# Qiyuan-Ge/PaintMind

Measured on AMD Instinct MI355X. Metric: 256x256 images/sec, 8-step MaskGIT decode (vit-s-vqgan), whole job, higher is better.
Workload: dtype bf16; 1 GPU; maskgit-uncond-12L-d512-T8; batch_per_gpu=64, topk=5, decode=every step (reference-equivalent work), parallelism=dp1 (independent images, no data-path collective), hip_graph=True, concurrent_micro_batches=2, dispatch_mode=AMD_DIRECT_DISPATCH=1 (default), rank_mode=False

## Files before the change

include/pmhip.h:

```cpp
#ifndef PMHIP_H
#define PMHIP_H

#include <stdint.h>

#ifdef __cplusplus
extern "C" {
#endif

#define PMHIP_ABI_VERSION 11

enum { PMHIP_OK = 0, PMHIP_EINVAL = 1, PMHIP_EHIP = 2, PMHIP_ENOMEM = 3, PMHIP_ESTATE = 4 };
enum { PMHIP_F32 = 0, PMHIP_BF16 = 1 };
enum { PMHIP_PART_Q = 0, PMHIP_PART_K = 1, PMHIP_PART_V = 2 };

typedef void* pmhip_stream;

int pmhip_abi_version(void);
const char* pmhip_last_error(void);
int pmhip_device_info(int device, int* cu_count, int* lds_bytes, char* arch, int arch_len);


int pmhip_gemm(int dtype, const void* A, int lda, const void* W, int ldw, const float* bias,
               const float* residual, int ldr, int res_rows, void* out, int ldo, int out_dtype,
               int M, int N, int K, pmhip_stream stream);
// ... 34 lines not shown
    const float* parts; int nparts; float eps;
} pmhip_lnfold;

int pmhip_gemm_ln(int dtype, const void* A, int lda, const void* W, int ldw, const float* bias, void* out,
                  int ldo, int out_dtype, int M, int N, int K, const pmhip_lnfold* ln, pmhip_stream stream);
int pmhip_gemm_swiglu_ln(int dtype, const void* A, int lda, const void* W12p, const float* b12p, void* out,
                         int ldo, int M, int Hp, int K, const pmhip_lnfold* ln, pmhip_stream stream);
int pmhip_gemm_heads_ln(int dtype, const void* A, int lda, const void* W, int ldw, int M, int K, int heads,
                        int tokens, int tokens_pad, int nparts, const int* part_kinds_host,
                        void* const* part_outs_host, float q_scale, const pmhip_lnfold* ln,
                        pmhip_stream stream);
int pmhip_lnfold_supported(int dtype, int epi_kind, int M, int N, int K);

int pmhip_gemm_softmax_stats(int dtype, const void* A, int lda, const void* W, int ldw, const float* bias, float* out, int ldo,
                             int M, int N, int K, const pmhip_lnfold* ln, float* block_stats, pmhip_stream stream);

int pmhip_attention(int dtype, const void* Q, const void* K, const void* Vt, void* out, int ldo,
                    int B, int heads, int Nq, int Nkv, int Nkv_pad, int use_exp2,
                    pmhip_stream stream);

int pmhip_attention_fallbacks(unsigned long long* count, int reset);

int pmhip_gemm_heads_dh(int dtype, const void* A, int lda, const void* W, int ldw, int M, int K, int heads, int dim_head,
                        int tokens, int tokens_pad, int nparts, const int* part_kinds_host,
                        void* const* part_outs_host, float q_scale, float* scratch, pmhip_stream stream);
int pmhip_attention_dh(int dtype, const void* Q, const void* K, const void* Vt, void* out, int ldo, int B, int heads,
                       int dim_head, int Nq, int Nkv, int Nkv_pad, int use_exp2, pmhip_stream stream);

int pmhip_layernorm(const float* x, const float* gamma, const float* beta, float eps, void* out,
                    int out_dtype, int M, int D, pmhip_stream stream);
// ... 175 lines not shown
                                   uint64_t image_base, float* imgs_out, int use_graph,
                                   pmhip_stream stream, float* imgs_host, size_t host_stride,
                                   pmhip_stream copy_stream, float guidance_scale);

#define PMHIP_SLOTS_GRAPH        1
#define PMHIP_SLOTS_KEEP_CONTEXT 2
int pmhip_pipeline_step_slots(pmhip_s2* s2, int64_t* ids, const float* context, int L, int B,
                              const pmhip_slot* slots_host, int flags,
                              int64_t* pred_out, float* score_out, pmhip_stream stream);

int pmhip_pipeline_step_slots_guided(pmhip_s2* s2, int64_t* ids, const float* context, int L, int B,
                                     const pmhip_slot* slots_host, const pmhip_slot_guide* guides_host, int flags,
                                     int64_t* pred_out, float* score_out, pmhip_stream stream);

int pmhip_s2_switches(const pmhip_s2* h);
int pmhip_vqgan_switches(const pmhip_vqgan* h);
int pmhip_s2_step0_shared(const pmhip_s2* h, int* fills, int* hits);
int pmhip_s2_slots_steps(const pmhip_s2* h, int* one_pass, int* two_pass);

int pmhip_timing_enable(int on);
int pmhip_timing_reset(void);
int pmhip_timing_get(const char* family, int* launches, double* total_ms);

#ifdef __cplusplus
}
#endif
#endif
```

paintmind_amd/_lib.py:

```python
import ctypes as C
import os

_HERE = os.path.dirname(os.path.abspath(__file__))
LIB_PATH = os.path.join(_HERE, "libpaintmind_hip.so")

PMHIP_OK = 0
PMHIP_EINVAL, PMHIP_EHIP, PMHIP_ENOMEM, PMHIP_ESTATE = 1, 2, 3, 4
F32, BF16 = 0, 1
PART_Q, PART_K, PART_V = 0, 1, 2
ABI_VERSION = 11
GENERATE_GRAPH, GENERATE_CONCURRENT_LANES, GENERATE_FROM_MASK = 1, 2, 4
SLOTS_GRAPH, SLOTS_KEEP_CONTEXT = 1, 2
SLOT_IDLE = 0x80000000

vp = C.c_void_p
i32 = C.c_int
f32 = C.c_float
u64 = C.c_uint64
u32 = C.c_uint32
i64 = C.c_int64


class LayerWeights(C.Structure):
    _fields_ = [(n, vp) for n in (
# ... 51 lines not shown
    "pmhip_gemm_swiglu": (i32, [i32, vp, i32, vp, vp, vp, i32, i32, i32, i32, vp]),
    "pmhip_gemm_heads": (i32, [i32, vp, i32, vp, i32, i32, i32, i32, i32, i32, i32, C.POINTER(i32),
                               C.POINTER(vp), f32, vp]),
    "pmhip_gemm_hilo": (i32, [vp, i32, vp, i32, vp, vp, vp, i32, i32, vp, vp, i32, i32, i32, i32, vp]),
    "pmhip_gemm_hilo_stats": (i32, [vp, i32, vp, i32, vp, vp, vp, i32, i32, vp, vp, i32, i32, i32, i32, vp, vp]),
    "pmhip_gemm_hilo_center": (i32, [vp, i32, vp, i32, vp, vp, vp, i32, i32, vp, vp, i32, i32, i32, i32, vp, vp, C.c_float, vp, i32, vp]),
    "pmhip_unshift_hilo": (i32, [vp, vp, vp, i32, i32, vp]),
    "pmhip_ln_coef_parts": (i32, [vp, i32, f32, vp, i32, vp]),
    "pmhip_layernorm_hilo": (i32, [vp, vp, vp, vp, f32, vp, i32, i32, i32, vp]),
    "pmhip_layernorm_to_hilo": (i32, [vp, vp, vp, f32, vp, vp, i32, i32, vp]),
    "pmhip_split_hilo": (i32, [vp, vp, vp, i32, i32, vp]),
    "pmhip_join_hilo": (i32, [vp, vp, vp, i32, i32, vp]),
    "pmhip_ln_coef": (i32, [vp, f32, vp, i32, i32, vp]),
    "pmhip_gemm_ln": (i32, [i32, vp, i32, vp, i32, vp, vp, i32, i32, i32, i32, i32, C.POINTER(LnFold), vp]),
    "pmhip_gemm_softmax_stats": (i32, [i32, vp, i32, vp, i32, vp, vp, i32, i32, i32, i32, C.POINTER(LnFold), vp, vp]),
    "pmhip_gemm_swiglu_ln": (i32, [i32, vp, i32, vp, vp, vp, i32, i32, i32, i32, C.POINTER(LnFold), vp]),
    "pmhip_gemm_heads_ln": (i32, [i32, vp, i32, vp, i32, i32, i32, i32, i32, i32, i32, C.POINTER(i32),
                                  C.POINTER(vp), f32, C.POINTER(LnFold), vp]),
    "pmhip_lnfold_supported": (i32, [i32, i32, i32, i32, i32]),
    "pmhip_attention": (i32, [i32, vp, vp, vp, vp, i32, i32, i32, i32, i32, i32, i32, vp]),
    "pmhip_attention_fallbacks": (i32, [C.POINTER(C.c_ulonglong), i32]),
    "pmhip_gemm_heads_dh": (i32, [i32, vp, i32, vp, i32, i32, i32, i32, i32, i32, i32, i32, C.POINTER(i32),
                                  C.POINTER(vp), f32, vp, vp]),
    "pmhip_attention_dh": (i32, [i32, vp, vp, vp, vp, i32, i32, i32, i32, i32, i32, i32, i32, vp]),
    "pmhip_layernorm": (i32, [vp, vp, vp, f32, vp, i32, i32, i32, vp]),
    "pmhip_patchify": (i32, [vp, vp, i32, i32, i32, i32, i32, i32, vp]),
    "pmhip_unpatchify_clamp": (i32, [vp, vp, i32, i32, i32, i32, i32, f32, f32, vp]),
    "pmhip_convert_pad": (i32, [vp, i32, vp, i32, i32, i32, vp]),
    "pmhip_add_rows": (i32, [vp, vp, i32, vp, i32, i32, vp]),
    "pmhip_guidance_combine": (i32, [vp, vp, C.c_float, vp, C.c_size_t, vp]),
# ... 74 lines not shown
```

paintmind_amd/csrc/engine.hip:

```cpp
#include <stdarg.h>
#include <string.h>

#include <algorithm>
#include <cmath>
#include <atomic>
#include <map>
#include <memory>
#include <mutex>

#include "common.h"

static thread_local std::string g_err;

void pm_set_error(const char* fmt, ...) {
    char buf[1024];
    va_list ap;
    va_start(ap, fmt);
    vsnprintf(buf, sizeof buf, fmt, ap);
    va_end(ap);
    g_err = buf;
}

extern "C" const char* pmhip_last_error(void) { return g_err.c_str(); }
extern "C" int pmhip_abi_version(void) { return PMHIP_ABI_VERSION; }
// ... 145 lines not shown
constexpr float kLog2e = 1.4426950408889634f;

struct CrossKV {
    const void* k = nullptr;
    const void* vt = nullptr;
    int L = 0, Lp = 0;
};

struct Switches {
    int overlap_rows = 65536;
    bool hilo = true;
    bool fold = true;
    int fold_rows_cap = 0;
    bool center = true;
    bool logits_stats = true;
    bool blocking_wait = false;
    static Switches from_env() {
        Switches w;
        const char* e = getenv("PMHIP_HILO");
        w.hilo = !(e && atoi(e) == 0);
        e = getenv("PMHIP_LN_UNFOLD");
        w.fold = !(e && atoi(e) != 0);
        e = getenv("PMHIP_FOLD_MAX_ROWS");
        w.fold_rows_cap = e ? atoi(e) : 0;
        e = getenv("PMHIP_HILO_CENTER");
        w.center = !(e && atoi(e) == 0);
        e = getenv("PMHIP_BLOCKING_WAIT");
        w.blocking_wait = e && atoi(e) != 0;
        e = getenv("PMHIP_DECODE_OVERLAP_MAX_ROWS");
        if (e) w.overlap_rows = atoi(e);
        w.logits_stats = pm_dev_knob("PMHIP_LOGITS_STATS", 1) != 0;
        return w;
    }
    int key() const { return (hilo ? 2 : 0) + (fold ? 1 : 0) + 4 + (center ? 8 : 0); }
};

struct FoldState {
    enum { kStale, kDeferred, kWritten } coef = kStale;
    bool parts = false;
    void produced(bool with_parts) { coef = kStale; parts = with_parts; }
    bool requested() { coef = parts ? kDeferred : kWritten; return !parts; }
    void consumed() { coef = kWritten; }
};

struct TowerBufs {
    float* x = nullptr;
// ... 506 lines not shown
    const size_t per = (size_t)B * heads * Lp * dh * es;
    unsigned char* kv;
    WS(h->ws, "ctx.kv", per * 2 * c.tower.depth, kv);
    float* split = nullptr;
    if (dh != 64) WS(h->ws, "ctx.split", (size_t)Mc * 2 * inner * 4, split);
    const int kinds[2] = {PMHIP_PART_K, PMHIP_PART_V};
    for (int l = 0; l < c.tower.depth; ++l) {
        void* outs[2] = {kv + per * (2 * l), kv + per * (2 * l + 1)};
        const unsigned char* wkv = reinterpret_cast<const unsigned char*>(h->layers[l].wqkv2) + (size_t)inner * dim * es;
        PM_TRY(pmhip_gemm_heads_dh(h->dtype, cp, dim, wkv, dim, Mc, dim, heads, dh, L, Lp, 2, kinds, outs, 1.0f, split, s));
        h->cross[l].k = outs[0]; h->cross[l].vt = outs[1]; h->cross[l].L = L; h->cross[l].Lp = Lp;
    }
    return PMHIP_OK;
}

int s2_tower(pmhip_s2* h, const void* tp, int B, float* logits, hipStream_t s, bool use_cross = true, float* block_stats = nullptr) {
    const auto& c = h->cfg;
    const int M = B * c.tokens, dim = c.tower.dim;
    TowerBufs tb;
    PM_TRY(alloc_tower(h->ws, h->sw, "s2", h->dtype, c.tower, B, c.tokens, tb, s));
    ResSrc pos;
    PM_TRY(pos_source(h->ws, "pos", tb.hilo, h->w.pos, c.tokens, dim, h->pos_split, pos, s));
    PM_TRY(residual_gemm(h->dtype, tb, tp, 64, h->w.tokproj_w, 64, h->w.tokproj_b, pos, M, dim, 64, s));
    for (int l = 0; l < c.tower.depth; ++l)
        PM_TRY(layer_forward(h->dtype, h->layers[l], c.tower, tb, B, c.tokens, true, use_cross ? &h->cross[l] : nullptr, s));
    if (tb.fold && h->w.logits_wf && fold_shape_ok(c.tokens, c.n_embed, dim))
        return folded_consumer(tb, M, c.tokens, dim, h->w.logits_c, h->w.logits_d, s, [&](int m0, int rows, const void* a, const pmhip_lnfold* ln) {
            float* out = logits + (size_t)m0 * c.n_embed;
            if (block_stats)
                return pmhip_gemm_softmax_stats(h->dtype, a, dim, h->w.logits_wf, dim, h->w.logits_b, out, c.n_embed, rows, c.n_embed, dim, ln,
                                                block_stats + (size_t)m0 * (c.n_embed / 64) * 2, s);
            return pmhip_gemm_ln(h->dtype, a, dim, h->w.logits_wf, dim, h->w.logits_b, out, c.n_embed, PMHIP_F32, rows, c.n_embed, dim, ln, s);
        });
    PM_TRY(tower_layernorm(h->dtype, tb, h->w.norm_g, h->w.norm_b, M, dim, s));
    if (block_stats)
        return pmhip_gemm_softmax_stats(h->dtype, tb.y, dim, h->w.logits_w, dim, h->w.logits_b, logits, c.n_embed, M, c.n_embed, dim, nullptr,
                                        block_stats, s);
    return pmhip_gemm(h->dtype, tb.y, dim, h->w.logits_w, dim, h->w.logits_b, nullptr, 0, 0, logits, c.n_embed, PMHIP_F32, M,
                      c.n_embed, dim, s);
}

struct StepBufs {
    float* logits = nullptr; float* lstats = nullptr;
    int64_t* pred = nullptr; float* score = nullptr;
};

int pred_bufs(pmhip_s2* s2, size_t M, StepBufs& b, hipStream_t s) {
    WS(s2->ws, "s2.pred", M * 8, b.pred);
    WS(s2->ws, "s2.score", M * 4, b.score);
    return PMHIP_OK;
}

int step_bufs(pmhip_s2* s2, int M, bool shared0, StepBufs& b, hipStream_t s) {
    const auto& c = s2->cfg;
    const size_t rows = shared0 ? c.tokens : M;
    WS(s2->ws, shared0 ? "s0.logits" : "s2.logits", rows * c.n_embed * 4, b.logits);
    b.lstats = nullptr;
    if (c.n_embed % 64 == 0 && s2->sw.logits_stats) WS(s2->ws, shared0 ? "s0.lstats" : "s2.lstats", rows * (c.n_embed / 64) * 8, b.lstats);
    return pred_bufs(s2, (size_t)M, b, s);
}

int tok_buf(pmhip_s2* s2, int M, void*& tp, hipStream_t s) {
    WS(s2->ws, "s2.tok", (size_t)M * 64 * dtype_size(s2->dtype), tp);
    return PMHIP_OK;
}

int step_tokens(pmhip_s2* s2, const int64_t* ids, int M, void*& tp, hipStream_t s) {
    PM_TRY(tok_buf(s2, M, tp, s));
    return pmhip_embed_rows(s2->w.tok_table, ids, tp, s2->dtype, 64, M, s2->cfg.n_embed + 1, s2->cfg.embed_dim, s);
}

int copy_aux(const StepBufs& b, size_t M, int64_t* pred_out, float* score_out, hipStream_t s) {
    if (pred_out) PM_HIP(hipMemcpyAsync(pred_out, b.pred, M * 8, hipMemcpyDeviceToDevice, s));
    if (score_out) PM_HIP(hipMemcpyAsync(score_out, b.score, M * 4, hipMemcpyDeviceToDevice, s));
    return PMHIP_OK;
}

int step_tower(pmhip_s2* s2, const int64_t* ids, int B, hipStream_t s, const float* guidance, const pmhip_slot* slots = nullptr,
               const pmhip_slot_guide* guides = nullptr) {
    const auto& c = s2->cfg;
    const int M = B * c.tokens;
    void* tp; StepBufs b;
    PM_TRY(step_tokens(s2, ids, M, tp, s));
    PM_TRY(step_bufs(s2, M, false, b, s));
    PM_TRY(s2_tower(s2, tp, B, b.logits, s, true, guidance ? nullptr : b.lstats));
    if (!guidance && !guides) return PMHIP_OK;
    float* uncond;
    WS(s2->ws, "s2.logits_u", (size_t)M * c.n_embed * 4, uncond);
    PM_TRY(s2_tower(s2, tp, B, uncond, s, false));
    if (guides) return pmhip_guidance_combine_slots(b.logits, uncond, guides, slots, c.tokens, b.logits, b.lstats, M, c.n_embed, s);
    if (b.lstats) return pmhip_guidance_combine_stats(b.logits, uncond, *guidance, b.logits, (size_t)M * c.n_embed, b.lstats, s);
    return pmhip_guidance_combine(b.logits, uncond, *guidance, b.logits, (size_t)M * c.n_embed, s);
}

int decode_pred(pmhip_s2* s2, pmhip_vqgan* vq, int B, float* img_out, hipStream_t s) {
    PM_REQUIRE(vq, "pipeline_sample: img_out requested without a vqgan handle");
    StepBufs b;
    PM_TRY(pred_bufs(s2, (size_t)B * s2->cfg.tokens, b, s));
    return vq_decode_indices(vq, b.pred, B, img_out, s);
}
// ... 218 lines not shown
    if (vq) img_elems = (size_t)B * vq->cfg.channels * vq->cfg.image_size * vq->cfg.image_size;
    int n_dec = 0;
    for (int t = 0; t < T; ++t) n_dec += c.decodes(t) ? 1 : 0;
    PM_REQUIRE(n_dec == 0 || (vq && (c.imgs_out || c.imgs_host)), "pipeline_generate: decode requested without vqgan / an image destination");
    PM_REQUIRE(!c.imgs_host || c.host_stride >= img_elems, "pipeline_generate: host_stride smaller than one image batch");
    const bool graph = (c.use_graph & PMHIP_GENERATE_GRAPH) && !g_pm_timing_on.load() && T <= PM_MAX_STEPS && !direct_dispatch_off();
    const bool from_mask = (c.use_graph & PMHIP_GENERATE_FROM_MASK) != 0;
    const bool share0 = from_mask && !c.context && !c.guidance && !g_pm_timing_on.load();
    const size_t n_ids = (size_t)B * s2->cfg.tokens;
    if (share0 && s2->s0_valid) {
        ++s2->s0_hits;
        if (s != s2->s0_stream) PM_HIP(hipStreamWaitEvent(s, s2->s0_ready.h, 0));
    }
    auto tower = [&](const int64_t* from, int t, hipStream_t on) -> int {
        if (share0 && t == 0) return step0_tower_once(s2, from, B, on);
        return step_tower(s2, from, B, on, c.guidance);
    };

    if (c.imgs_host) {
        const unsigned evflags = hipEventDisableTiming | (s2->sw.blocking_wait ? hipEventBlockingSync : 0u);
        hipEvent_t e;
        PM_TRY(s2->host_copied.get(evflags, e));
        if ((int)s2->img_ready.size() < n_dec) s2->img_ready.resize(n_dec);
        for (int d = 0; d < n_dec; ++d) PM_TRY(s2->img_ready[d].get(evflags, e));
    }
    float* gimgs = nullptr;
    if (n_dec && (graph || !c.imgs_out)) {
        WS(s2->ws, "gen.imgs", (size_t)n_dec * img_elems * 4 + 16, gimgs);
        if (s2->host_copy_pending) { PM_HIP(hipStreamWaitEvent(s, s2->host_copied.h, 0)); s2->host_copy_pending = false; }
    }
    HostDelivery out{c, s, cs, img_elems, n_dec, gimgs != nullptr};
// ... 32 lines not shown

    std::string key = "B" + std::to_string(B) + "T" + std::to_string(T) + "k" + std::to_string(c.topk) + "L" +
                      std::to_string(c.context ? c.L : 0) + "v" + std::to_string(vq ? vq->uid : 0) + "f" +
                      std::to_string(s2->sw.key() * 16 + (vq ? vq->sw.key() : 0));
    if (c.guidance) {
        unsigned bits;
        memcpy(&bits, c.guidance, 4);
        key += "g" + std::to_string(bits);
    }
    key += "d";
    for (int t = 0; t < T; ++t) key += c.decodes(t) ? '1' : '0';
    const bool overlap = vq && n_dec > 0 && s2->sw.overlap_rows > 0 && (long long)B * s2->cfg.tokens <= s2->sw.overlap_rows &&
                         !(c.use_graph & PMHIP_GENERATE_CONCURRENT_LANES);
    const std::vector<Unit> units = plan_units(c, overlap);
    key += overlap ? "o1" : "o0";
    if (from_mask) key += "m";
    hipStream_t side = nullptr;
    hipEvent_t ev_fork = nullptr, ev_join = nullptr;
    if (overlap) {
        PM_TRY(s2->side_stream.get(hipStreamNonBlocking, side));
        PM_TRY(s2->ev_fork.get(hipEventDisableTiming, ev_fork));
        PM_TRY(s2->ev_join.get(hipEventDisableTiming, ev_join));
    }

    auto run_unit = [&](hipStream_t on, size_t i) -> int {
        const Unit& u = units[i];
        bool need_join = false;
        if (u.decode_first >= 0) {
            float* img = gimgs + (size_t)u.decode_first * img_elems;
            if (u.t1 > u.t0) {
// ... 123 lines not shown
extern "C" int pmhip_s2_slots_steps(const pmhip_s2* h, int* one_pass, int* two_pass) {
    PM_REQUIRE(h, "s2_slots_steps: null handle");
    if (one_pass) *one_pass = h->slots_one_pass;
    if (two_pass) *two_pass = h->slots_two_pass;
    return PMHIP_OK;
}

extern "C" int pmhip_s2_step0_shared(const pmhip_s2* h, int* fills, int* hits) {
    PM_REQUIRE(h, "s2_step0_shared: null handle");
    if (fills) *fills = h->s0_fills;
    if (hits) *hits = h->s0_hits;
    return PMHIP_OK;
}

extern "C" int pmhip_s2_switches(const pmhip_s2* h) {
    return h ? h->sw.key() + (h->sw.blocking_wait ? 16 : 0) + (direct_dispatch_off() ? 32 : 0) : -1;
}
extern "C" int pmhip_vqgan_switches(const pmhip_vqgan* h) { return h ? h->sw.key() + (h->sw.blocking_wait ? 16 : 0) : -1; }
```

paintmind_amd/csrc/gemm.hip:

```cpp
#include <stdlib.h>

#include "gemm_common.h"

using namespace pmgemm;

int pm_gemm256_supported(const GemmParams& p, int dtype, int epi, int out_dtype);
int pm_gemm256_launch(const GemmParams& p, int epi, int out_dtype, hipStream_t s);
int pm_gemm2b_supported(const GemmParams& p, int dtype, int epi, int out_dtype);
int pm_gemm2b_launch(const GemmParams& p, int epi, int out_dtype, hipStream_t s);

namespace {

constexpr int BM = 128, BN = 128;
constexpr int TILE_BYTES = 128 * ROWB;
constexpr int STAGE_BYTES = 2 * TILE_BYTES;
constexpr int THREADS = 256;

template <typename T, int CH = 4>
__device__ __forceinline__ void stage_tile(const T* __restrict__ base, int ld, int row0, int rows_total,
                                           int k0, unsigned char* lds_tile, int wave, int lane) {
#pragma unroll
    for (int i = 0; i < CH; ++i) {
        const int chunk = wave * CH + i;
        const int r = chunk * 8 + (lane >> 3);
// ... 262 lines not shown
        if (ln->parts) {
            if (deep) { p.ln_parts = ln->parts; p.ln_nparts = ln->nparts; p.ln_eps = ln->eps; p.ln_coef_out = const_cast<float*>(ln->coef); }
            else PM_TRY(pmhip_ln_coef_parts(ln->parts, ln->nparts, ln->eps, const_cast<float*>(ln->coef), p.M, stream));
        }
        if (small) return launch_bf16<EPI, true>(p, out_dtype, deep, s);
        return pm_gemm256_launch(p, EPI, out_dtype, s);
    }
    if (use2b(p, dtype, EPI, out_dtype)) return pm_gemm2b_launch(p, EPI, out_dtype, s);
    if (use256(p, dtype, EPI, out_dtype)) return pm_gemm256_launch(p, EPI, out_dtype, s);
    if (dtype == PMHIP_F32) return launch<float, EPI, float>(p, false, s);
    return launch_bf16<EPI, false>(p, out_dtype, deep128(p), s);
}

int gemm_impl(int dtype, const void* A, int lda, const void* W, int ldw, const float* bias,
                          const float* residual, int ldr, int res_rows, void* out, int ldo, int out_dtype,
                          int M, int N, int K, const pmhip_lnfold* ln, pmhip_stream stream, float* block_stats = nullptr) {
    GemmParams p{};
    p.A = A; p.W = W; p.bias = bias; p.residual = residual; p.out = out;
    p.block_stats = block_stats;
    PM_REQUIRE(!block_stats || (out_dtype == PMHIP_F32 && !residual && N % 64 == 0),
               "gemm_softmax_stats: block statistics need an f32 output without a residual and N=%d a multiple of 64", N);
    p.lda = lda; p.ldw = ldw; p.ldr = ldr; p.res_rows = res_rows > 0 ? res_rows : M; p.ldo = ldo;
    p.M = M; p.N = N; p.K = K;
    PM_TRY(check_common(p, dtype));
    PM_REQUIRE(out, "gemm: null out");
    PM_REQUIRE(N % 4 == 0 && ldo % 4 == 0, "gemm: N=%d and ldo=%d must be multiples of 4", N, ldo);
    PM_REQUIRE(ldo >= N, "gemm: ldo=%d is smaller than N=%d (rows of out would overlap)", ldo, N);
    PM_REQUIRE(!residual || ldr % 4 == 0, "gemm: ldr must be a multiple of 4");
    PM_REQUIRE(!residual || ldr >= N, "gemm: ldr=%d is smaller than N=%d (rows of the residual would overlap)", ldr, N);
    PM_REQUIRE(!residual || out_dtype == PMHIP_F32, "gemm: a residual needs an f32 output (the residual stream is f32)");
    PM_REQUIRE(out_dtype == PMHIP_F32 || out_dtype == dtype, "gemm: out dtype must be f32 or the compute dtype");
    PM_REQUIRE(out_dtype == PMHIP_F32 || ldo % 8 == 0, "gemm: bf16 output needs ldo to be a multiple of 8");
    return dispatch<EPI_STD>(p, dtype, out_dtype, ln, stream);
}
// ... 50 lines not shown
                          center_extra, shift, shift_mode);
}

extern "C" int pmhip_gemm_ln(int dtype, const void* A, int lda, const void* W, int ldw, const float* bias, void* out, int ldo,
                             int out_dtype, int M, int N, int K, const pmhip_lnfold* ln, pmhip_stream stream) {
    PM_REQUIRE(ln, "gemm_ln: null fold descriptor");
    return gemm_impl(dtype, A, lda, W, ldw, bias, nullptr, 0, 0, out, ldo, out_dtype, M, N, K, ln, stream);
}

extern "C" int pmhip_gemm_softmax_stats(int dtype, const void* A, int lda, const void* W, int ldw, const float* bias, float* out, int ldo,
                                        int M, int N, int K, const pmhip_lnfold* ln, float* block_stats, pmhip_stream stream) {
    PM_REQUIRE(block_stats, "gemm_softmax_stats: null statistics buffer");
    return gemm_impl(dtype, A, lda, W, ldw, bias, nullptr, 0, 0, out, ldo, PMHIP_F32, M, N, K, ln, stream, block_stats);
}

extern "C" int pmhip_lnfold_supported(int dtype, int epi_kind, int M, int N, int K) {
    return dtype == PMHIP_BF16 && epi_kind >= 0 && epi_kind <= 2 && pm_lnfold_shape_ok(M, N, K, K, K) ? 1 : 0;
}

static int gemm_swiglu_impl(int dtype, const void* A, int lda, const void* W12p, const float* b12p,
                                 void* out, int ldo, int M, int Hp, int K, const pmhip_lnfold* ln, pmhip_stream stream) {
    GemmParams p{};
    p.A = A; p.W = W12p; p.bias = b12p; p.out = out;
    p.lda = lda; p.ldw = K; p.ldo = ldo; p.M = M; p.N = 2 * Hp; p.K = K;
    p.fast_math = (dtype == PMHIP_BF16);
    PM_TRY(check_common(p, dtype));
    PM_REQUIRE(Hp % 64 == 0, "gemm_swiglu: padded hidden width %d must be a multiple of 64", Hp);
    PM_REQUIRE(b12p && out && ldo % 8 == 0, "gemm_swiglu: bias/out required, ldo multiple of 8");
    PM_REQUIRE(ldo >= Hp, "gemm_swiglu: ldo=%d is smaller than Hp=%d (rows of out would overlap)", ldo, Hp);
    return dispatch<EPI_SWIGLU>(p, dtype, dtype, ln, stream);
// ... 50 lines not shown
```

paintmind_amd/csrc/gemm_common.h:

```cpp
#pragma once
#include "common.h"

namespace pmgemm {

constexpr int ROWB = 128;
constexpr int ESTRIDE = 68;
constexpr int EPI_WAVE_BYTES = 8192;

enum { EPI_STD = 0, EPI_SWIGLU = 1, EPI_HEADS = 2 };

struct GemmParams {
    const void* A; const void* W;
    const float* bias; const float* residual;
    void* out;
    int lda, ldw, ldr, res_rows, ldo;
    int M, N, K;
    int heads, tokens, tokens_pad, inner;
    int kinds[3];
    void* outs[3];
    float q_scale;
    int fast_math;
    int chunk;
    const bf16_t* res_lo; bf16_t* out_lo;
    float* row_stats;
    const float* center_coef; float center_extra; float* shift; int shift_mode;
    const float* ln_coef;
    const float* ln_c; const float* ln_d;
    const float* ln_parts; int ln_nparts; float ln_eps; float* ln_coef_out;
    float* block_stats;
};

inline int gemm_family(const GemmParams& p, int epi, bool two_wg = false) {
    if (epi == EPI_HEADS) return FAM_GEMM_HEADS;
    if (epi == EPI_SWIGLU) return FAM_GEMM_SWIGLU;
    if (p.residual || p.out_lo) return two_wg ? FAM_GEMM_RESID2B : FAM_GEMM_RESID;
    return FAM_GEMM;
}

__device__ __forceinline__ int xcd_remap(int bid, int nblocks) {
    const int q = nblocks >> 3, r = nblocks & 7;
    const int xcd = bid & 7, local = bid >> 3;
    const int base = (xcd < r) ? xcd * (q + 1) : r * (q + 1) + (xcd - r) * q;
    return base + local;
}
// ... 183 lines not shown
            }
        }
    }
    constexpr bool GATE_IN_REGS = (EPI == EPI_SWIGLU) && sizeof(OutT) == 2;
    float4 sb[4] = {};
    if constexpr (GATE_IN_REGS) {
        const float* b1 = p.bias + nw + g * 4;
        sb[0] = *reinterpret_cast<const float4*>(b1);      sb[1] = *reinterpret_cast<const float4*>(b1 + 16);
        sb[2] = *reinterpret_cast<const float4*>(b1 + 32); sb[3] = *reinterpret_cast<const float4*>(b1 + 48);
    } else if constexpr (EPI == EPI_SWIGLU) {
        const int q = lane & 3;
        const float* b1 = p.bias + nw + (q >> 1) * 32 + (q & 1) * 8;
        sb[0] = *reinterpret_cast<const float4*>(b1);      sb[1] = *reinterpret_cast<const float4*>(b1 + 4);
        sb[2] = *reinterpret_cast<const float4*>(b1 + 16); sb[3] = *reinterpret_cast<const float4*>(b1 + 20);
    }
    __builtin_amdgcn_s_waitcnt(0x0F70);
    hook();
    if constexpr (GATE_IN_REGS && FULL) {
        constexpr int RS = 80, BUFB = 2048;
        auto stage = [&](int mi) {
            unsigned char* row = eraw + (mi & 1) * BUFB + l15 * RS;
            *reinterpret_cast<uint2*>(row + g * 8) = make_uint2(
                pack_bf16x2(silu_mul_fast(acc[mi][0][0] + sb[0].x, acc[mi][1][0] + sb[1].x),
                            silu_mul_fast(acc[mi][0][1] + sb[0].y, acc[mi][1][1] + sb[1].y)),
                pack_bf16x2(silu_mul_fast(acc[mi][0][2] + sb[0].z, acc[mi][1][2] + sb[1].z),
                            silu_mul_fast(acc[mi][0][3] + sb[0].w, acc[mi][1][3] + sb[1].w)));
            *reinterpret_cast<uint2*>(row + 32 + g * 8) = make_uint2(
                pack_bf16x2(silu_mul_fast(acc[mi][2][0] + sb[2].x, acc[mi][3][0] + sb[3].x),
                            silu_mul_fast(acc[mi][2][1] + sb[2].y, acc[mi][3][1] + sb[3].y)),
                pack_bf16x2(silu_mul_fast(acc[mi][2][2] + sb[2].z, acc[mi][3][2] + sb[3].z),
                            silu_mul_fast(acc[mi][2][3] + sb[2].w, acc[mi][3][3] + sb[3].w)));
        };
// ... 217 lines not shown
                            q2 += dpp_mov<0xB1>(q2); q2 += dpp_mov<0x4E>(q2); q2 += dpp_mov<0x141>(q2);
                            if ((lane & 7) == 0)
                                *reinterpret_cast<float2*>(p.row_stats + ((size_t)mm * (p.N >> 6) + (nw >> 6)) * 2) = make_float2(sm, q2);
                        }
                        continue;
                    }
                    if constexpr (sizeof(OutT) == 4 && RES != 0) {
                        if (RES == 1 || p.residual) {
                            float4 rr;
                            if constexpr (PIPE_RES) rr = rcur[it];
                            else if constexpr (NPRE > 1) rr = rpre[mi * ITERS + it];
                            else rr = *reinterpret_cast<const float4*>(p.residual + (size_t)(mm % p.res_rows) * p.ldr + ncol);
                            v[0] += rr.x; v[1] += rr.y; v[2] += rr.z; v[3] += rr.w;
                        }
                    }
                    st_row<NT>(reinterpret_cast<OutT*>(p.out) + (size_t)mm * p.ldo + ncol, v);
                    if constexpr (sizeof(OutT) == 4) {
                        if (p.block_stats) {
                            const float2 st = softmax_block_stat(v[0], v[1], v[2], v[3]);
                            if ((lane & (LPR - 1)) == 0)
                                *reinterpret_cast<float2*>(p.block_stats + ((size_t)mm * (p.N >> 6) + (nw >> 6)) * 2) = st;
                        }
                    }
                }
            }
        } else if constexpr (EPI == EPI_SWIGLU) {
            const int erow = lane >> 2, m = mbase + erow;
            if (FULL || m < p.M) {
                const int q = lane & 3;
                const int c1 = (q >> 1) * 32 + (q & 1) * 8;
                const float* e1 = ebuf + erow * ESTRIDE + c1;
                const float4 a0 = *reinterpret_cast<const float4*>(e1), a1 = *reinterpret_cast<const float4*>(e1 + 4);
                const float4 g0 = *reinterpret_cast<const float4*>(e1 + 16), g1 = *reinterpret_cast<const float4*>(e1 + 20);
                const float4 ba0 = sb[0], ba1 = sb[1], bg0 = sb[2], bg1 = sb[3];
                float h[8];
                h[0] = silu_mul(a0.x + ba0.x, g0.x + bg0.x, p.fast_math); h[1] = silu_mul(a0.y + ba0.y, g0.y + bg0.y, p.fast_math);
                h[2] = silu_mul(a0.z + ba0.z, g0.z + bg0.z, p.fast_math); h[3] = silu_mul(a0.w + ba0.w, g0.w + bg0.w, p.fast_math);
                h[4] = silu_mul(a1.x + ba1.x, g1.x + bg1.x, p.fast_math); h[5] = silu_mul(a1.y + ba1.y, g1.y + bg1.y, p.fast_math);
// ... 39 lines not shown
```

paintmind_amd/csrc/rowops.hip:

```cpp
#include <algorithm>

#include "common.h"

namespace {

constexpr int THREADS = 256;

template <typename OutT, int NV4>
__global__ __launch_bounds__(THREADS) void layernorm_kernel(const float* __restrict__ x, const float* __restrict__ gamma,
                                                            const float* __restrict__ beta, float eps,
                                                            OutT* __restrict__ out, int M, int D) {
    const int lane = threadIdx.x & 63;
    const int row = blockIdx.x * (THREADS / 64) + (threadIdx.x >> 6);
    if (row >= M) return;
    const float* xr = x + (size_t)row * D;
    OutT* orow = out + (size_t)row * D;
    const float invD = 1.0f / (float)D;
    if constexpr (NV4 > 0) {
        float4 v[NV4];
        float s = 0.f;
#pragma unroll
        for (int i = 0; i < NV4; ++i) {
            v[i] = *reinterpret_cast<const float4*>(xr + (i * 64 + lane) * 4);
            s += (v[i].x + v[i].y) + (v[i].z + v[i].w);
// ... 396 lines not shown
    PM_HIP(hipGetLastError());
    return PMHIP_OK;
}

extern "C" int pmhip_ln_coef_parts(const float* row_stats, int nparts, float eps, float* coef, int M, pmhip_stream stream) {
    PM_REQUIRE(row_stats && coef, "ln_coef_parts: null pointer");
    PM_REQUIRE(M > 0 && nparts > 0 && nparts <= 16, "ln_coef_parts: nparts=%d must be in [1,16] (D = 64 * nparts <= 1024)", nparts);
    hipStream_t s = (hipStream_t)stream;
    PmTimer tm(FAM_LAYERNORM, s);
    hipLaunchKernelGGL(ln_coef_parts_kernel, dim3(ceil_div(M * 8, THREADS)), dim3(THREADS), 0, s,
                       reinterpret_cast<const float2*>(row_stats), nparts, eps, reinterpret_cast<float2*>(coef), M);
    PM_HIP(hipGetLastError());
    return PMHIP_OK;
}

extern "C" int pmhip_patchify(const float* img, void* out, int out_dtype, int B, int C, int H, int W, int P,
                              pmhip_stream stream) {
    PM_REQUIRE(img && out, "patchify: null pointer");
    PM_REQUIRE(B > 0 && C > 0 && P % 8 == 0 && H % P == 0 && W % P == 0, "patchify: bad geometry (P must be a multiple of 8)");
    hipStream_t s = (hipStream_t)stream;
    const size_t total = (size_t)B * (H / P) * (W / P) * (C * P * P / 8);
    PmTimer tm(FAM_ROWOPS, s);
    if (out_dtype == PMHIP_F32)
        hipLaunchKernelGGL((patchify_kernel<float>), dim3(grid_for(total)), dim3(THREADS), 0, s, img, (float*)out, B, C, H, W, P);
    else
        hipLaunchKernelGGL((patchify_kernel<bf16_t>), dim3(grid_for(total)), dim3(THREADS), 0, s, img, (bf16_t*)out, B, C, H, W, P);
    PM_HIP(hipGetLastError());
    return PMHIP_OK;
}

// ... 102 lines not shown
```

paintmind_amd/engine.py:

```python
import ctypes as C

import numpy as np
import torch

from . import _lib, ops, packing
from ._lib import LayerWeights, S2Cfg, S2Weights, TowerCfg, VqganCfg, VqganWeights, check
from .ops import _p, pm_dtype, round_up, stream_ptr


def _f32(t):
    return t.detach().float().contiguous()


class _Keep:

    def __init__(self):
        self.tensors = []

    def __call__(self, t):
        self.tensors.append(t)
        return C.c_void_p(t.data_ptr())


def _pack_layer(layer, dtype, keep, stage2):
# ... 29 lines not shown
                lw.wqkv2_f, lw.qkv2_c, lw.qkv2_d = fold(packing.pack_qkv(a2.to_q, a2.to_k, a2.to_v, torch.float32), layer.norm2)
        lw.w12p_f, lw.w12_c, lw.w12_d = fold(packing.pack_w12(layer.ffnet.w12, torch.float32)[0], ffn_norm)
    return lw, hp


def _pack_tower(layers, dtype, keep, stage2):
    arr = (LayerWeights * len(layers))()
    hp = 0
    for i, layer in enumerate(layers):
        arr[i], hp = _pack_layer(layer, dtype, keep, stage2)
    return arr, hp


def _switch_dict(bits):
    return {"ln_fold": bool(bits & 1), "hilo": bool(bits & 2), "ln_stats": bool(bits & 4), "hilo_center": bool(bits & 8),
            "blocking_wait": bool(bits & 16), "graph_replay_off": bool(bits & 32)}


class VqganEngine:

    @property
    def switches(self):
        return _switch_dict(self.lib.pmhip_vqgan_switches(self.handle))

    def __init__(self, model, dtype):
        self.lib = _lib.load()
        dev = next(model.parameters()).device
        if dev.type != "cuda":
            raise _lib.PmhipError("paintmind_amd needs the model on a ROCm device (model.to('cuda')); no CPU fallback")
        self.device, self.dtype = dev, dtype
        keep = self.keep = _Keep()
# ... 99 lines not shown
        x = x.to(self.device, torch.float32).contiguous()
        B = x.shape[0]
        img = self._new_img(B)
        with torch.cuda.device(self.device):
            check(self.lib.pmhip_vqgan_decoder_forward(self.handle, _p(x), B, _p(img), stream_ptr(self.device)),
                  "pmhip_vqgan_decoder_forward")
        return img


class S2Engine:

    @property
    def switches(self):
        return _switch_dict(self.lib.pmhip_s2_switches(self.handle))

    def step0_shared(self):
        fills, hits = C.c_int(0), C.c_int(0)
        check(self.lib.pmhip_s2_step0_shared(self.handle, C.byref(fills), C.byref(hits)), "pmhip_s2_step0_shared")
        return fills.value, hits.value

    def __init__(self, transformer, codebook, mask_token, dtype):
        self.lib = _lib.load()
        dev = next(transformer.parameters()).device
        if dev.type != "cuda":
            raise _lib.PmhipError("paintmind_amd needs the model on a ROCm device (model.to('cuda')); no CPU fallback")
        self.device, self.dtype = dev, dtype
        keep = self.keep = _Keep()
        tr = transformer
        layers = list(tr.layers)
        with torch.cuda.device(dev):
# ... 151 lines not shown
```

paintmind_amd/ops.py:

```python
import ctypes as C
import math

import torch

from . import _lib
from ._lib import BF16, F32, PART_K, PART_Q, PART_V, check

_TORCH2PM = {torch.float32: F32, torch.bfloat16: BF16}


def pm_dtype(dt):
    try:
        return _TORCH2PM[dt]
    except KeyError:
        raise TypeError(f"paintmind_amd computes in float32 or bfloat16, not {dt}") from None


def _dev(*tensors):
    dev = None
    for t in tensors:
        if t is None:
            continue
        if not t.is_cuda:
            raise _lib.PmhipError(
# ... 215 lines not shown
def gemm_softmax_stats(x, w, bias=None, fold=None):
    dev = _dev(x, w, bias)
    lib = _lib.load()
    M, K = x.shape
    N = w.shape[0]
    if N % 64:
        raise ValueError("gemm_softmax_stats: N must be a multiple of 64")
    out = torch.empty(M, N, device=dev, dtype=torch.float32)
    stats = torch.empty(M, N // 64, 2, device=dev, dtype=torch.float32)
    ln = _lnfold(*fold) if fold is not None else None
    with torch.cuda.device(dev):
        check(lib.pmhip_gemm_softmax_stats(pm_dtype(x.dtype), _p(x), x.stride(0), _p(w), w.stride(0), _p(bias), _p(out), N, M, N, K,
                                           C.byref(ln) if ln is not None else None, _p(stats), stream_ptr(dev)),
              "pmhip_gemm_softmax_stats")
    return out, stats


def gemm_swiglu_ln(xb, w12pg, b12p, coef, c, d, parts=None):
    dev = _dev(xb, w12pg, b12p)
    lib = _lib.load()
    M, K = xb.shape
    Hp = w12pg.shape[0] // 2
    out = torch.empty(M, Hp, device=dev, dtype=xb.dtype)
    ln = _lnfold(coef, c, d, parts)
    with torch.cuda.device(dev):
        check(lib.pmhip_gemm_swiglu_ln(pm_dtype(xb.dtype), _p(xb), xb.stride(0), _p(w12pg), _p(b12p), _p(out), Hp, M, Hp, K,
                                       C.byref(ln), stream_ptr(dev)), "pmhip_gemm_swiglu_ln")
    return out


# ... 324 lines not shown
```

Baseline: 536.5 images/s.

## Prune logits stores for vocabulary blocks that cannot reach the top-k

Splits the logits GEMM with softmax statistics into a head pass over the first 2048 vocabulary columns and a tail pass over the rest. Between them, a small kernel takes the k-th largest head block maximum per row as a threshold. In the tail pass, 64-column blocks whose maximum falls below that threshold still write their softmax statistics but skip writing their fp32 logits. This is meant to cut the large fp32 logits write traffic during top-k sampling, at the cost of an extra launch and a split GEMM. It relies on downstream consumers reading only blocks selected through the statistics.

```diff
diff --git a/include/pmhip.h b/include/pmhip.h
--- a/include/pmhip.h
+++ b/include/pmhip.h
@@ -72,6 +72,11 @@
 
 int pmhip_gemm_softmax_stats(int dtype, const void* A, int lda, const void* W, int ldw, const float* bias, float* out, int ldo,
                              int M, int N, int K, const pmhip_lnfold* ln, float* block_stats, pmhip_stream stream);
+
+int pmhip_gemm_softmax_stats_cols(int dtype, const void* A, int lda, const void* W, int ldw, const float* bias, float* out, int ldo,
+                                  int M, int N, int K, const pmhip_lnfold* ln, float* block_stats, int col0, int ncols,
+                                  const float* store_thr, pmhip_stream stream);
+int pmhip_block_kth_max(const float* block_stats, int nblk, int nhead, int k, float* thr, int M, pmhip_stream stream);
 
 int pmhip_attention(int dtype, const void* Q, const void* K, const void* Vt, void* out, int ldo,
                     int B, int heads, int Nq, int Nkv, int Nkv_pad, int use_exp2,
@@ -277,6 +282,7 @@
                                      int64_t* pred_out, float* score_out, pmhip_stream stream);
 
 int pmhip_s2_switches(const pmhip_s2* h);
+int pmhip_s2_set_logits_prune(pmhip_s2* h, int on);
 int pmhip_vqgan_switches(const pmhip_vqgan* h);
 int pmhip_s2_step0_shared(const pmhip_s2* h, int* fills, int* hits);
 int pmhip_s2_slots_steps(const pmhip_s2* h, int* one_pass, int* two_pass);
diff --git a/paintmind_amd/_lib.py b/paintmind_amd/_lib.py
--- a/paintmind_amd/_lib.py
+++ b/paintmind_amd/_lib.py
@@ -89,6 +89,9 @@
     "pmhip_ln_coef": (i32, [vp, f32, vp, i32, i32, vp]),
     "pmhip_gemm_ln": (i32, [i32, vp, i32, vp, i32, vp, vp, i32, i32, i32, i32, i32, C.POINTER(LnFold), vp]),
     "pmhip_gemm_softmax_stats": (i32, [i32, vp, i32, vp, i32, vp, vp, i32, i32, i32, i32, C.POINTER(LnFold), vp, vp]),
+    "pmhip_gemm_softmax_stats_cols": (i32, [i32, vp, i32, vp, i32, vp, vp, i32, i32, i32, i32, C.POINTER(LnFold), vp, i32, i32, vp, vp]),
+    "pmhip_block_kth_max": (i32, [vp, i32, i32, i32, vp, i32, vp]),
+    "pmhip_s2_set_logits_prune": (i32, [vp, i32]),
     "pmhip_gemm_swiglu_ln": (i32, [i32, vp, i32, vp, vp, vp, i32, i32, i32, i32, C.POINTER(LnFold), vp]),
     "pmhip_gemm_heads_ln": (i32, [i32, vp, i32, vp, i32, i32, i32, i32, i32, i32, i32, C.POINTER(i32),
                                   C.POINTER(vp), f32, C.POINTER(LnFold), vp]),
diff --git a/paintmind_amd/csrc/engine.hip b/paintmind_amd/csrc/engine.hip
--- a/paintmind_amd/csrc/engine.hip
+++ b/paintmind_amd/csrc/engine.hip
@@ -183,6 +183,7 @@
     int fold_rows_cap = 0;
     bool center = true;
     bool logits_stats = true;
+    bool logits_prune = true;
     bool blocking_wait = false;
     static Switches from_env() {
         Switches w;
@@ -199,6 +200,7 @@
         e = getenv("PMHIP_DECODE_OVERLAP_MAX_ROWS");
         if (e) w.overlap_rows = atoi(e);
         w.logits_stats = pm_dev_knob("PMHIP_LOGITS_STATS", 1) != 0;
+        w.logits_prune = pm_dev_knob("PMHIP_LOGITS_PRUNE", 1) != 0;
         return w;
     }
     int key() const { return (hilo ? 2 : 0) + (fold ? 1 : 0) + 4 + (center ? 8 : 0); }
@@ -735,7 +737,29 @@
     return PMHIP_OK;
 }
 
-int s2_tower(pmhip_s2* h, const void* tp, int B, float* logits, hipStream_t s, bool use_cross = true, float* block_stats = nullptr) {
+constexpr int LOGITS_HEAD = 2048;
+int logits_prune_k(const pmhip_s2* h, int topk) {
+    const auto& c = h->cfg;
+    if (!h->sw.logits_prune || !h->sw.logits_stats || h->dtype != PMHIP_BF16 || topk < 1 || topk > 8) return 0;
+    if (c.n_embed % 256 || c.n_embed < 2 * LOGITS_HEAD || c.tokens % 256 || c.tower.dim % 64 || c.tower.dim < 128) return 0;
+    return topk;
+}
+
+int logits_gemm_stats(pmhip_s2* h, const void* a, const void* w, float* out, int rows, const pmhip_lnfold* ln, float* block_stats, float* thr,
+                      int prune_k, hipStream_t s) {
+    const auto& c = h->cfg;
+    const int V = c.n_embed, dim = c.tower.dim;
+    if (!prune_k) return pmhip_gemm_softmax_stats(h->dtype, a, dim, w, dim, h->w.logits_b, out, V, rows, V, dim, ln, block_stats, s);
+    PM_TRY(pmhip_gemm_softmax_stats_cols(h->dtype, a, dim, w, dim, h->w.logits_b, out, V, rows, V, dim, ln, block_stats, 0, LOGITS_HEAD, nullptr, s));
+    PM_TRY(pmhip_block_kth_max(block_stats, V / 64, LOGITS_HEAD / 64, prune_k, thr, rows, s));
+    pmhip_lnfold tail{};
+    if (ln) { tail = *ln; tail.parts = nullptr; tail.nparts = 0; }
+    return pmhip_gemm_softmax_stats_cols(h->dtype, a, dim, w, dim, h->w.logits_b, out, V, rows, V, dim, ln ? &tail : nullptr, block_stats,
+                                         LOGITS_HEAD, V - LOGITS_HEAD, thr, s);
+}
+
+int s2_tower(pmhip_s2* h, const void* tp, int B, float* logits, hipStream_t s, bool use_cross = true, float* block_stats = nullptr,
+             float* thr = nullptr, int prune_k = 0) {
     const auto& c = h->cfg;
     const int M = B * c.tokens, dim = c.tower.dim;
     TowerBufs tb;
@@ -749,20 +773,19 @@
         return folded_consumer(tb, M, c.tokens, dim, h->w.logits_c, h->w.logits_d, s, [&](int m0, int rows, const void* a, const pmhip_lnfold* ln) {
             float* out = logits + (size_t)m0 * c.n_embed;
             if (block_stats)
-                return pmhip_gemm_softmax_stats(h->dtype, a, dim, h->w.logits_wf, dim, h->w.logits_b, out, c.n_embed, rows, c.n_embed, dim, ln,
-                                                block_stats + (size_t)m0 * (c.n_embed / 64) * 2, s);
+                return logits_gemm_stats(h, a, h->w.logits_wf, out, rows, ln, block_stats + (size_t)m0 * (c.n_embed / 64) * 2,
+                                         thr ? thr + m0 : nullptr, prune_k, s);
             return pmhip_gemm_ln(h->dtype, a, dim, h->w.logits_wf, dim, h->w.logits_b, out, c.n_embed, PMHIP_F32, rows, c.n_embed, dim, ln, s);
         });
     PM_TRY(tower_layernorm(h->dtype, tb, h->w.norm_g, h->w.norm_b, M, dim, s));
-    if (block_stats)
-        return pmhip_gemm_softmax_stats(h->dtype, tb.y, dim, h->w.logits_w, dim, h->w.logits_b, logits, c.n_embed, M, c.n_embed, dim, nullptr,
-                                        block_stats, s);
+    if (block_stats) return logits_gemm_stats(h, tb.y, h->w.logits_w, logits, M, nullptr, block_stats, thr, prune_k, s);
     return pmhip_gemm(h->dtype, tb.y, dim, h->w.logits_w, dim, h->w.logits_b, nullptr, 0, 0, logits, c.n_embed, PMHIP_F32, M,
                       c.n_embed, dim, s);
 }
 
 struct StepBufs {
     float* logits = nullptr; float* lstats = nullptr;
+    float* lthr = nullptr;
     int64_t* pred = nullptr; float* score = nullptr;
 };
 
@@ -778,6 +801,8 @@
     WS(s2->ws, shared0 ? "s0.logits" : "s2.logits", rows * c.n_embed * 4, b.logits);
     b.lstats = nullptr;
     if (c.n_embed % 64 == 0 && s2->sw.logits_stats) WS(s2->ws, shared0 ? "s0.lstats" : "s2.lstats", rows * (c.n_embed / 64) * 8, b.lstats);
+    b.lthr = nullptr;
+    if (!shared0 && b.lstats && logits_prune_k(s2, 1)) WS(s2->ws, "s2.lthr", rows * 4, b.lthr);
     return pred_bufs(s2, (size_t)M, b, s);
 }
 
@@ -798,13 +823,14 @@
 }
 
 int step_tower(pmhip_s2* s2, const int64_t* ids, int B, hipStream_t s, const float* guidance, const pmhip_slot* slots = nullptr,
-               const pmhip_slot_guide* guides = nullptr) {
+               const pmhip_slot_guide* guides = nullptr, int prune_topk = 0) {
     const auto& c = s2->cfg;
     const int M = B * c.tokens;
     void* tp; StepBufs b;
     PM_TRY(step_tokens(s2, ids, M, tp, s));
     PM_TRY(step_bufs(s2, M, false, b, s));
-    PM_TRY(s2_tower(s2, tp, B, b.logits, s, true, guidance ? nullptr : b.lstats));
+    const int prune_k = (guidance || guides || slots || !b.lstats || !b.lthr) ? 0 : logits_prune_k(s2, prune_topk);
+    PM_TRY(s2_tower(s2, tp, B, b.logits, s, true, guidance ? nullptr : b.lstats, b.lthr, prune_k));
     if (!guidance && !guides) return PMHIP_OK;
     float* uncond;
     WS(s2->ws, "s2.logits_u", (size_t)M * c.n_embed * 4, uncond);
@@ -1053,7 +1079,7 @@
     }
     auto tower = [&](const int64_t* from, int t, hipStream_t on) -> int {
         if (share0 && t == 0) return step0_tower_once(s2, from, B, on);
-        return step_tower(s2, from, B, on, c.guidance);
+        return step_tower(s2, from, B, on, c.guidance, nullptr, nullptr, c.topk);
     };
 
     if (c.imgs_host) {
@@ -1116,6 +1142,7 @@
                          !(c.use_graph & PMHIP_GENERATE_CONCURRENT_LANES);
     const std::vector<Unit> units = plan_units(c, overlap);
     key += overlap ? "o1" : "o0";
+    key += s2->sw.logits_prune ? "p1" : "p0";
     if (from_mask) key += "m";
     hipStream_t side = nullptr;
     hipEvent_t ev_fork = nullptr, ev_join = nullptr;
@@ -1269,6 +1296,11 @@
 }
 
 extern "C" int pmhip_s2_switches(const pmhip_s2* h) {
-    return h ? h->sw.key() + (h->sw.blocking_wait ? 16 : 0) + (direct_dispatch_off() ? 32 : 0) : -1;
+    return h ? h->sw.key() + (h->sw.blocking_wait ? 16 : 0) + (direct_dispatch_off() ? 32 : 0) + (h->sw.logits_prune ? 0 : 64) : -1;
+}
+extern "C" int pmhip_s2_set_logits_prune(pmhip_s2* h, int on) {
+    PM_REQUIRE(h, "s2_set_logits_prune: null handle");
+    h->sw.logits_prune = on != 0;
+    return PMHIP_OK;
 }
 extern "C" int pmhip_vqgan_switches(const pmhip_vqgan* h) { return h ? h->sw.key() + (h->sw.blocking_wait ? 16 : 0) : -1; }
diff --git a/paintmind_amd/csrc/gemm.hip b/paintmind_amd/csrc/gemm.hip
--- a/paintmind_amd/csrc/gemm.hip
+++ b/paintmind_amd/csrc/gemm.hip
@@ -300,10 +300,11 @@
 
 int gemm_impl(int dtype, const void* A, int lda, const void* W, int ldw, const float* bias,
                           const float* residual, int ldr, int res_rows, void* out, int ldo, int out_dtype,
-                          int M, int N, int K, const pmhip_lnfold* ln, pmhip_stream stream, float* block_stats = nullptr) {
+                          int M, int N, int K, const pmhip_lnfold* ln, pmhip_stream stream, float* block_stats = nullptr,
+                          int stats_nblk = 0, int stats_blk0 = 0, const float* store_thr = nullptr) {
     GemmParams p{};
     p.A = A; p.W = W; p.bias = bias; p.residual = residual; p.out = out;
-    p.block_stats = block_stats;
+    p.block_stats = block_stats; p.stats_nblk = stats_nblk; p.stats_blk0 = stats_blk0; p.store_thr = store_thr;
     PM_REQUIRE(!block_stats || (out_dtype == PMHIP_F32 && !residual && N % 64 == 0),
                "gemm_softmax_stats: block statistics need an f32 output without a residual and N=%d a multiple of 64", N);
     p.lda = lda; p.ldw = ldw; p.ldr = ldr; p.res_rows = res_rows > 0 ? res_rows : M; p.ldo = ldo;
@@ -384,6 +385,27 @@
     return gemm_impl(dtype, A, lda, W, ldw, bias, nullptr, 0, 0, out, ldo, PMHIP_F32, M, N, K, ln, stream, block_stats);
 }
 
+extern "C" int pmhip_gemm_softmax_stats_cols(int dtype, const void* A, int lda, const void* W, int ldw, const float* bias, float* out,
+                                             int ldo, int M, int N, int K, const pmhip_lnfold* ln, float* block_stats, int col0, int ncols,
+                                             const float* store_thr, pmhip_stream stream) {
+    PM_REQUIRE(block_stats && W && out, "gemm_softmax_stats_cols: null pointer");
+    PM_REQUIRE(dtype == PMHIP_F32 || dtype == PMHIP_BF16, "gemm_softmax_stats_cols: bad dtype %d", dtype);
+    PM_REQUIRE(N > 0 && N % 64 == 0 && ldo >= N, "gemm_softmax_stats_cols: N=%d must be a multiple of 64 and ldo=%d at least N", N, ldo);
+    PM_REQUIRE(col0 >= 0 && col0 % 256 == 0 && ncols > 0 && ncols % 64 == 0 && col0 <= N - ncols,
+               "gemm_softmax_stats_cols: columns [%d, %d + %d) must start at a multiple of 256, be whole 64-column blocks and lie inside N=%d",
+               col0, col0, ncols, N);
+    PM_REQUIRE(ldw >= K && K > 0, "gemm_softmax_stats_cols: ldw=%d is smaller than K=%d (rows of W would overlap)", ldw, K);
+    pmhip_lnfold sub{};
+    if (ln) {
+        PM_REQUIRE(ln->c && ln->d, "gemm_ln: null fold pointer");
+        sub = *ln; sub.c += col0; sub.d += col0;
+    }
+    const size_t es = dtype == PMHIP_BF16 ? 2 : 4;
+    return gemm_impl(dtype, A, lda, reinterpret_cast<const unsigned char*>(W) + (size_t)col0 * ldw * es, ldw, bias ? bias + col0 : nullptr,
+                     nullptr, 0, 0, out + col0, ldo, PMHIP_F32, M, ncols, K, ln ? &sub : nullptr, stream, block_stats, N / 64, col0 / 64,
+                     store_thr);
+}
+
 extern "C" int pmhip_lnfold_supported(int dtype, int epi_kind, int M, int N, int K) {
     return dtype == PMHIP_BF16 && epi_kind >= 0 && epi_kind <= 2 && pm_lnfold_shape_ok(M, N, K, K, K) ? 1 : 0;
 }
diff --git a/paintmind_amd/csrc/gemm_common.h b/paintmind_amd/csrc/gemm_common.h
--- a/paintmind_amd/csrc/gemm_common.h
+++ b/paintmind_amd/csrc/gemm_common.h
@@ -28,6 +28,8 @@
     const float* ln_c; const float* ln_d;
     const float* ln_parts; int ln_nparts; float ln_eps; float* ln_coef_out;
     float* block_stats;
+    int stats_nblk, stats_blk0;
+    const float* store_thr;
 };
 
 inline int gemm_family(const GemmParams& p, int epi, bool two_wg = false) {
@@ -241,8 +243,28 @@
         sb[0] = *reinterpret_cast<const float4*>(b1);      sb[1] = *reinterpret_cast<const float4*>(b1 + 4);
         sb[2] = *reinterpret_cast<const float4*>(b1 + 16); sb[3] = *reinterpret_cast<const float4*>(b1 + 20);
     }
+    constexpr bool THR = (EPI == EPI_STD) && sizeof(OutT) == 4 && RES <= 0;
+    constexpr int THR_OFF = 16 * ESTRIDE;
+    [[maybe_unused]] const bool pruned = THR && p.store_thr && p.block_stats;
+    [[maybe_unused]] float thr_up[(MI * 16 + 63) / 64] = {};
+    if constexpr (THR) {
+        if (pruned) {
+#pragma unroll
+            for (int i = 0; i < (MI * 16 + 63) / 64; ++i) {
+                const int r = i * 64 + lane;
+                if (r < MI * 16 && (FULL || mwave + r < p.M)) thr_up[i] = p.store_thr[mwave + r];
+            }
+        }
+    }
     __builtin_amdgcn_s_waitcnt(0x0F70);
     hook();
+    if constexpr (THR) {
+        if (pruned) {
+#pragma unroll
+            for (int i = 0; i < (MI * 16 + 63) / 64; ++i)
+                if (i * 64 + lane < MI * 16) ebuf[THR_OFF + i * 64 + lane] = thr_up[i];
+        }
+    }
     if constexpr (GATE_IN_REGS && FULL) {
         constexpr int RS = 80, BUFB = 2048;
         auto stage = [&](int mi) {
@@ -490,14 +512,19 @@
                             v[0] += rr.x; v[1] += rr.y; v[2] += rr.z; v[3] += rr.w;
                         }
                     }
-                    st_row<NT>(reinterpret_cast<OutT*>(p.out) + (size_t)mm * p.ldo + ncol, v);
+                    bool keep = true;
                     if constexpr (sizeof(OutT) == 4) {
                         if (p.block_stats) {
                             const float2 st = softmax_block_stat(v[0], v[1], v[2], v[3]);
+                            const int nblk = p.stats_nblk ? p.stats_nblk : (p.N >> 6);
                             if ((lane & (LPR - 1)) == 0)
-                                *reinterpret_cast<float2*>(p.block_stats + ((size_t)mm * (p.N >> 6) + (nw >> 6)) * 2) = st;
+                                *reinterpret_cast<float2*>(p.block_stats + ((size_t)mm * nblk + p.stats_blk0 + (nw >> 6)) * 2) = st;
+                            if constexpr (THR) {
+                                if (pruned) keep = !(st.x < ebuf[THR_OFF + mi * 16 + r]);
+                            }
                         }
                     }
+                    if (keep) st_row<NT>(reinterpret_cast<OutT*>(p.out) + (size_t)mm * p.ldo + ncol, v);
                 }
             }
         } else if constexpr (EPI == EPI_SWIGLU) {
diff --git a/paintmind_amd/csrc/rowops.hip b/paintmind_amd/csrc/rowops.hip
--- a/paintmind_amd/csrc/rowops.hip
+++ b/paintmind_amd/csrc/rowops.hip
@@ -434,6 +434,33 @@
     return PMHIP_OK;
 }
 
+__global__ __launch_bounds__(THREADS) void block_kth_max_kernel(const float2* __restrict__ stats, int nblk, int nhead, int k,
+                                                                float* __restrict__ thr, int M) {
+    const int row = blockIdx.x * (THREADS / 64) + (threadIdx.x >> 6), lane = threadIdx.x & 63;
+    if (row >= M) return;
+    float v = lane < nhead ? stats[(size_t)row * nblk + lane].x : -INFINITY;
+    float m = -INFINITY;
+    for (int i = 0; i < k; ++i) {
+        m = wave_max(v);
+        const unsigned long long at = __ballot(v == m);
+        if (at == 0) break;
+        if (lane == __ffsll((long long)at) - 1) v = -INFINITY;
+    }
+    if (lane == 0) thr[row] = m;
+}
+
+extern "C" int pmhip_block_kth_max(const float* block_stats, int nblk, int nhead, int k, float* thr, int M, pmhip_stream stream) {
+    PM_REQUIRE(block_stats && thr, "block_kth_max: null pointer");
+    PM_REQUIRE(M > 0 && nblk > 0 && nhead >= 1 && nhead <= 64 && nhead <= nblk && k >= 1 && k <= nhead,
+               "block_kth_max: need 1 <= k=%d <= nhead=%d <= min(64, nblk=%d)", k, nhead, nblk);
+    hipStream_t s = (hipStream_t)stream;
+    PmTimer tm(FAM_ROWOPS, s);
+    hipLaunchKernelGGL(block_kth_max_kernel, dim3(ceil_div(M, THREADS / 64)), dim3(THREADS), 0, s,
+                       reinterpret_cast<const float2*>(block_stats), nblk, nhead, k, thr, M);
+    PM_HIP(hipGetLastError());
+    return PMHIP_OK;
+}
+
 extern "C" int pmhip_patchify(const float* img, void* out, int out_dtype, int B, int C, int H, int W, int P,
                               pmhip_stream stream) {
     PM_REQUIRE(img && out, "patchify: null pointer");
diff --git a/paintmind_amd/engine.py b/paintmind_amd/engine.py
--- a/paintmind_amd/engine.py
+++ b/paintmind_amd/engine.py
@@ -67,7 +67,7 @@
 
 def _switch_dict(bits):
     return {"ln_fold": bool(bits & 1), "hilo": bool(bits & 2), "ln_stats": bool(bits & 4), "hilo_center": bool(bits & 8),
-            "blocking_wait": bool(bits & 16), "graph_replay_off": bool(bits & 32)}
+            "blocking_wait": bool(bits & 16), "graph_replay_off": bool(bits & 32), "logits_prune": not bits & 64}
 
 
 class VqganEngine:
@@ -197,6 +197,9 @@
     def switches(self):
         return _switch_dict(self.lib.pmhip_s2_switches(self.handle))
 
+    def set_logits_prune(self, on):
+        check(self.lib.pmhip_s2_set_logits_prune(self.handle, int(bool(on))), "pmhip_s2_set_logits_prune")
+
     def step0_shared(self):
         fills, hits = C.c_int(0), C.c_int(0)
         check(self.lib.pmhip_s2_step0_shared(self.handle, C.byref(fills), C.byref(hits)), "pmhip_s2_step0_shared")
diff --git a/paintmind_amd/ops.py b/paintmind_amd/ops.py
--- a/paintmind_amd/ops.py
+++ b/paintmind_amd/ops.py
@@ -253,6 +253,36 @@
                                            C.byref(ln) if ln is not None else None, _p(stats), stream_ptr(dev)),
               "pmhip_gemm_softmax_stats")
     return out, stats
+
+
+def gemm_softmax_stats_cols(x, w, out, stats, col0, ncols, bias=None, fold=None, thr=None):
+    dev = _dev(x, w, bias, out, stats, thr)
+    lib = _lib.load()
+    M, K = x.shape
+    N = w.shape[0]
+    if (out.dtype != torch.float32 or out.dim() != 2 or tuple(out.shape) != (M, N) or out.stride(1) != 1 or stats.dtype != torch.float32
+            or not stats.is_contiguous() or tuple(stats.shape) != (M, N // 64, 2) or N % 64):
+        raise ValueError("gemm_softmax_stats_cols: out must be fp32 [M, N] with unit column stride, stats contiguous fp32 [M, N/64, 2]")
+    if thr is not None and (thr.dtype != torch.float32 or not thr.is_contiguous() or tuple(thr.shape) != (M,)):
+        raise ValueError("gemm_softmax_stats_cols: thr must be a contiguous fp32 [M] tensor")
+    ln = _lnfold(*fold) if fold is not None else None
+    with torch.cuda.device(dev):
+        check(lib.pmhip_gemm_softmax_stats_cols(pm_dtype(x.dtype), _p(x), x.stride(0), _p(w), w.stride(0), _p(bias), _p(out), out.stride(0),
+                                                M, N, K, C.byref(ln) if ln is not None else None, _p(stats), int(col0), int(ncols),
+                                                _p(thr), stream_ptr(dev)), "pmhip_gemm_softmax_stats_cols")
+    return out, stats
+
+
+def block_kth_max(stats, nhead, k):
+    dev = _dev(stats)
+    lib = _lib.load()
+    if stats.dtype != torch.float32 or not stats.is_contiguous() or stats.dim() != 3 or stats.shape[2] != 2:
+        raise ValueError("block_kth_max: stats must be a contiguous fp32 [M, nblk, 2] tensor")
+    M, nblk = stats.shape[0], stats.shape[1]
+    thr = torch.empty(M, device=dev, dtype=torch.float32)
+    with torch.cuda.device(dev):
+        check(lib.pmhip_block_kth_max(_p(stats), nblk, int(nhead), int(k), _p(thr), M, stream_ptr(dev)), "pmhip_block_kth_max")
+    return thr
 
 
 def gemm_swiglu_ln(xb, w12pg, b12p, coef, c, d, parts=None):
```

Measured after the change: 533.4 images/s. About the same (-0.6%).
